# hitbc/panSVR

Hardware: AMD Instinct MI355X
Metric: signal reads realigned/sec (150 bp PE); bit-exact CIGAR vs CPU ref (higher is better)
Workload: dtype u8/int32 (2-bit k-mers, 8-bit DP deltas, 32-bit scores); 1 GPU; configs[1]: 1000000 synthetic 150 bp PE signal read pairs per GPU vs 10000-anchor SV reference (11.8 Mbp), `panSVR aln` hot path; pairs_per_gpu=1000000, engines_per_gpu=1, in_process_rebases=0, index_hbm_bytes=2713674320, index_distribution=every rank uploads its own copy from host memory

## Files before the change

### pansvr_amd/csrc/dp_plan.h

```cpp
#pragma once
#include <stdint.h>
#include <string.h>
#include <algorithm>
#include <vector>
#include "../../include/psvr_engine.h"

#if defined(__HIPCC__)
#define PSVR_HD __host__ __device__ __forceinline__
#else
#define PSVR_HD inline
#endif

namespace psvr {

#define PSVR_DP_NUM_LDS_CLASSES 13
#define PSVR_DP_MAX_LDS (160 * 1024)
PSVR_HD int dp_lds_class_bytes(int cls)
{
	const int t[PSVR_DP_NUM_LDS_CLASSES] = {2048, 4096, 6144, 8192, 12288, 16384, 24576, 32768, 49152, 65536, 98304, 131072, PSVR_DP_MAX_LDS};
	return t[cls];
}
PSVR_HD int dp_lds_class(long long need)
{
	int cls = 0;
// ... 23 lines not shown
}

#define PSVR_DP_STRIP 16
#define PSVR_DP_TINY_MAX 16
#define PSVR_DP_PG_THRESHOLD 4096
static const int kDpWaves = 4;
static const int kDpLongLen = 8000;
static const int kDpMaxSeqLen = 1 << 28;
static const int kDpTinySmallLds = 4096;
PSVR_HD bool dp_band_never_binds(int qlen, int tlen, int w) { return qlen <= w && tlen <= w + 1; }
PSVR_HD int dp_band_w(int qlen, int tlen, int w) { return w < 0 ? (qlen > tlen ? qlen : tlen) : w; }
PSVR_HD int dp_n_col(int qlen, int tlen, int w_in)
{
	int w = dp_band_w(qlen, tlen, w_in);
	int n_col = qlen < tlen ? qlen : tlen;
	n_col = ((n_col < w + 1 ? n_col : w + 1) + 15) / 16 + 1;
	return n_col;
}
PSVR_HD long long dp_reg_lds_need(int qlen, int tlen, int w_in)
{
	return (long long)((qlen + 16 + 15) & ~15) + (long long)(qlen + tlen - 1) * dp_n_col(qlen, tlen, w_in) * 16 + 16;
}
PSVR_HD long long dp_p_bytes(int qlen, int tlen, int w_in)
{
	return ((long long)(qlen + tlen - 1) * dp_n_col(qlen, tlen, w_in) + 1) * 16;
}
PSVR_HD constexpr int dp_lds_kernel_need(int qlen, int tlen, int variant)
{
	int T = (tlen + 15) / 16 * 16, QL = (qlen + 15) / 16 * 16;
	int narr = variant == 0 ? 7 : 5;
	int img = narr * T + T + QL + 16;
	return ((img + 15) & ~15) + 4 * T;
}
static_assert(dp_lds_kernel_need(kDpLongLen, kDpLongLen, 0) <= PSVR_DP_MAX_LDS, "the general kernel's LDS holds every problem that is not long");
PSVR_HD long long dp_hbm_img_off(int qlen, int tlen, int w_in, bool with_cigar)
{
	return with_cigar ? (dp_p_bytes(qlen, tlen, w_in) + 255) & ~255LL : 0;
}
PSVR_HD long long dp_hbm_img_bytes(int qlen, int tlen, int variant)
{
	const long long T = (tlen + 15LL) / 16 * 16, QL = (qlen + 15LL) / 16 * 16;
	return (((variant == 0 ? 8 : 6) * T + QL + 16 + 15) & ~15LL) + 4 * T;
}

struct DpParams {
	int32_t m;
	int32_t q, e, q2, e2;
	int32_t qe_pre;
	int32_t sc_mch, sc_mis, sc_N, m1;
	int32_t w, zdrop, end_bonus, flag;
	int32_t long_thres, long_diff;
	int32_t skip;
	int32_t nowrap_ok;
	int8_t  mat[25];
};
inline bool make_dp_params(const psvr_ksw_params_t *par, int variant, DpParams *P)
{
	memset(P, 0, sizeof *P);
	int m = par->m, q = par->q, e = par->e, q2 = par->q2, e2 = par->e2;
	if (m > 5 || m < 0) return false;
	P->m = m;
	P->qe_pre = q + e;
	memcpy(P->mat, par->mat, 25);
	P->w = par->w, P->zdrop = par->zdrop, P->end_bonus = par->end_bonus, P->flag = par->flag;
	if (variant == 0) {
		if (m <= 1) { P->skip = 1; return true; }
		if (q2 + e2 < q + e) { int t = q; q = q2, q2 = t, t = e, e = e2, e2 = t; }
	} else {
		if (m <= 0) { P->skip = 1; return true; }
		q2 = q, e2 = e;
	}
	P->q = q, P->e = e, P->q2 = q2, P->e2 = e2;
	P->sc_mch = par->mat[0], P->sc_mis = par->mat[1];
	P->sc_N = par->mat[m * m - 1] == 0 ? (int8_t)(-e2) : par->mat[m * m - 1];
	if (variant == 1) P->sc_N = par->mat[m * m - 1] == 0 ? (int8_t)(-e) : par->mat[m * m - 1];
	P->m1 = m - 1;
	int min_sc = par->mat[1];
	for (int t = 1; t < m * m; ++t) min_sc = std::min<int>(min_sc, par->mat[t]);
	if (-min_sc > 2 * (q + e)) { P->skip = 1; return true; }
	{
		int max_sc = par->mat[0];
		for (int t = 1; t < m * m; ++t) max_sc = std::max<int>(max_sc, par->mat[t]);
		int g = std::max(q + e, q2 + e2);
		const bool boundary_is_the_recurrences = e > e2 || (e == e2 && q == q2);
		P->nowrap_ok = (max_sc + 3 * g + std::max(-min_sc, 0) <= 127) && q >= 0 && e >= 0 && q2 >= 0 && e2 >= 0 && boundary_is_the_recurrences;
	}
	if (variant == 0) {
		int lt = e != e2 ? (q2 - q) / (e - e2) - 1 : 0;
		if (q2 + e2 + lt * e2 > q + e + lt * e) ++lt;
		P->long_thres = lt;
		P->long_diff = lt * (e - e2) - (q2 - q) - e2;
	}
	return true;
}
inline bool dp_zdrop_inert(const DpParams &P)
{
	return P.e2 == 0 && (P.zdrop < 0 || P.zdrop >= 2 * P.q2 + (P.qe_pre - (P.q + P.e))) && !(P.flag & PSVR_EZ_EXTZ_ONLY);
}
PSVR_HD bool dp_fast_ok(int flag, int variant) { return variant == 0 && (flag & ~(PSVR_EZ_EXTZ_ONLY | PSVR_EZ_REV_CIGAR | PSVR_EZ_SCORE_ONLY)) == 0; }
PSVR_HD bool dp_tiny_ok(const DpParams &P, bool fast_ok) { return fast_ok && P.nowrap_ok && !P.skip && (P.w < 0 || P.w >= PSVR_DP_TINY_MAX); }

struct DpRoute {
	int kind, need;
	int64_t slab;
};
PSVR_HD DpRoute dp_route(int qlen, int tlen, int w, bool fast_ok, int variant, bool skip, bool tiny_ok, bool team_ok, bool with_cigar)
{
	const bool is_long = qlen > kDpLongLen || tlen > kDpLongLen;
	DpRoute R{1, 0, 0};
	if (skip || (!is_long && (qlen <= 0 || tlen <= 0))) return R;
	const bool dirs = with_cigar || !is_long;
	const int64_t p_slab = dirs ? (dp_p_bytes(qlen, tlen, w) + 255) & ~(int64_t)255 : 0;
	if (!is_long) {
		if (tiny_ok && qlen <= PSVR_DP_TINY_MAX && tlen <= PSVR_DP_TINY_MAX) { R.kind = PSVR_DP_KIND_TINY, R.need = (qlen + tlen - 1) * 512; return R; }
		if (tiny_ok && team_ok && dp_band_never_binds(qlen, tlen, dp_band_w(qlen, tlen, w)) && tlen <= PSVR_DP_STRIP * PSVR_DP_NUM_LDS_CLASSES) {
			R.kind = PSVR_DP_KIND_STRIP, R.need = dp_lds_class_bytes((tlen + PSVR_DP_STRIP - 1) / PSVR_DP_STRIP - 1);
			return R;
		}
		const int T = (tlen + 15) / 16 * 16;
		if (fast_ok && T <= 320) {
			const long long n = dp_reg_lds_need(qlen, tlen, w);
			if (n <= PSVR_DP_PG_THRESHOLD) { R.kind = (T + 63) / 64, R.need = (int)n; return R; }
			R.kind = 5 + (T + 63) / 64, R.need = ((qlen + 16 + 15) & ~15) + 16, R.slab = p_slab;
			return R;
		}
	}
	if (fast_ok) {
		const int wf = dp_band_w(qlen, tlen, w), sh = qlen < tlen ? qlen : tlen;
		const int span = (wf < sh - 1 ? wf : sh - 1) + 33;
		const long long ring_need = ((qlen + 16 + 15) & ~15LL) + ((tlen + 15) & ~15LL) + 16;
		if (span <= 256 && ring_need <= PSVR_DP_MAX_LDS) {
			const bool four = (long long)dp_lds_class_bytes(dp_lds_class(ring_need)) * kDpWaves <= PSVR_DP_MAX_LDS;
			R.kind = span <= 192 ? (four ? PSVR_DP_KIND_RING3 : PSVR_DP_KIND_RING1_3) : (four ? PSVR_DP_KIND_RING4 : PSVR_DP_KIND_RING1_4);
			R.need = (int)ring_need, R.slab = p_slab;
			return R;
		}
	}
	if (is_long) {
		R.kind = PSVR_DP_KIND_HBM;
		R.slab = dp_hbm_img_off(qlen, tlen, w, with_cigar) + ((dp_hbm_img_bytes(qlen, tlen, variant) + 255) & ~(int64_t)255);
		return R;
	}
	R.kind = 0, R.need = dp_lds_kernel_need(qlen, tlen, variant), R.slab = p_slab;
	return R;
}

static constexpr int kDpTeamLanes = 2, kDpTeamCpl = 8;
PSVR_HD int dp_team_lanes(int n_strips16) { return kDpTeamLanes; }
PSVR_HD unsigned long long dp_team_ws_bytes(int qmax, int n_strips16, int lanes, int cpl = kDpTeamCpl)
{
	const int sw = cpl * lanes, pb = 64 / lanes, n_strips = (n_strips16 * 16 + sw - 1) / sw;
	return (unsigned long long)(64 * cpl) * n_strips * (qmax + sw - 1) + (unsigned long long)pb * 20 * (qmax + sw * n_strips + 1);
}
PSVR_HD unsigned long long dp_team_waves(int cls, unsigned long long count) { return (count * dp_team_lanes(cls + 1) + 63) / 64; }
PSVR_HD unsigned long long dp_team_wave_ws(int cls, int qmax) { return dp_team_ws_bytes(qmax > 0 ? qmax : 1, cls + 1, dp_team_lanes(cls + 1)); }
PSVR_HD unsigned long long dp_team_class_ws(int cls, unsigned long long count, int qmax) { return dp_team_waves(cls, count) * dp_team_wave_ws(cls, qmax); }

PSVR_HD int dp_kind_order(int k)
{
	const int t[PSVR_DP_NUM_HOST_KINDS] = {17, 16, 15, 0, 14, 13, 10, 9, 8, 7, 6, 5, 4, 3, 2, 1, PSVR_DP_KIND_TINY, PSVR_DP_KIND_STRIP};
	return t[k];
}
static const int kDpPlanClasses = PSVR_DP_NUM_LDS_CLASSES, kDpPlanKinds = PSVR_DP_NUM_KINDS, kDpPlanTeamKind = PSVR_DP_KIND_STRIP, kDpPlanQBins = 200;
static const int kDpPlanTeam0 = 256;
static const int kDpPlanBuckets = kDpPlanTeam0 + kDpPlanClasses * kDpPlanQBins;
static const int kDpPlanOtherSlots = (kDpPlanKinds - 1) * kDpPlanClasses;
static const int kDpPlanSlots = kDpPlanOtherSlots + kDpPlanClasses * kDpPlanQBins;
static_assert(PSVR_DP_NUM_HOST_KINDS * PSVR_DP_NUM_LDS_CLASSES <= kDpPlanTeam0, "a count per (kind, class) below the team buckets");
PSVR_HD int dp_plan_bucket(int kind, int cls, int qlen)
{
	if (kind == kDpPlanTeamKind) return kDpPlanTeam0 + cls * kDpPlanQBins + (qlen < 1 ? 0 : qlen > kDpPlanQBins ? kDpPlanQBins - 1 : qlen - 1);
	return kind * kDpPlanClasses + cls;
}
PSVR_HD int dp_plan_slot_bucket(int k)
{
	if (k < kDpPlanOtherSlots) return dp_kind_order(PSVR_DP_NUM_HOST_KINDS - PSVR_DP_NUM_KINDS + k / kDpPlanClasses) * kDpPlanClasses + (kDpPlanClasses - 1 - k % kDpPlanClasses);
	k -= kDpPlanOtherSlots;
	return kDpPlanTeam0 + (kDpPlanClasses - 1 - k / kDpPlanQBins) * kDpPlanQBins + (kDpPlanQBins - 1 - k % kDpPlanQBins);
}
inline long long dp_plan_starts(const unsigned int *hist, long long *start)
{
	long long acc = 0;
	for (int b = 0; b < kDpPlanBuckets; ++b) start[b] = 0;
	for (int k = 0; k < kDpPlanSlots; ++k) { const int b = dp_plan_slot_bucket(k); start[b] = acc, acc += hist[b]; }
	return acc;
}

struct DpLaunch {
	int kind, cls;
	long long first, count;
	int qmax;
};
inline std::vector<DpLaunch> dp_launch_list(const unsigned long long *cnt, const unsigned long long *team_cnt, const unsigned long long *team_qmax, bool merge_tiny)
{
	std::vector<DpLaunch> ls;
	long long acc = 0;
	for (int ko = 0; ko < PSVR_DP_NUM_HOST_KINDS; ++ko)
		for (int cls = PSVR_DP_NUM_LDS_CLASSES - 1; cls >= 0; --cls) {
			const int kind = dp_kind_order(ko);
			const bool team = kind == PSVR_DP_KIND_STRIP;
			const long long n = (long long)(team ? team_cnt[cls] : cnt[kind * PSVR_DP_NUM_LDS_CLASSES + cls]);
			if (!n) continue;
			const bool joins = merge_tiny && kind == PSVR_DP_KIND_TINY && !ls.empty() && ls.back().kind == kind &&
			                   (dp_lds_class_bytes(ls.back().cls) > kDpTinySmallLds) == (dp_lds_class_bytes(cls) > kDpTinySmallLds);
			if (joins) ls.back().count += n;
			else ls.push_back(DpLaunch{kind, cls, acc, n, team ? (int)team_qmax[cls] : 0});
			acc += n;
		}
	return ls;
}

struct DpHostPlan {
	std::vector<int32_t> idx;
	std::vector<int64_t> poff;
	std::vector<DpLaunch> launches;
	int64_t slab_bytes = 0, ws_bytes = 0;
};
inline DpHostPlan dp_plan_host(int64_t n, const int32_t *qlen, const int32_t *tlen, const DpParams &P, int variant)
{
	DpHostPlan out;
	const bool fast_ok = dp_fast_ok(P.flag, variant), tiny_ok = dp_tiny_ok(P, fast_ok), with_cigar = !(P.flag & PSVR_EZ_SCORE_ONLY);
	unsigned long long cnt[PSVR_DP_NUM_HOST_KINDS * PSVR_DP_NUM_LDS_CLASSES] = {}, qmax[PSVR_DP_NUM_LDS_CLASSES] = {};
	std::vector<int> slot(n);
	out.poff.assign(n, 0);
	for (int64_t i = 0; i < n; ++i) {
		const DpRoute R = dp_route(qlen[i], tlen[i], P.w, fast_ok, variant, P.skip != 0, tiny_ok, true, with_cigar);
		if (R.slab) out.poff[i] = out.slab_bytes, out.slab_bytes += R.slab;
		const int cls = dp_lds_class(R.need);
		++cnt[slot[i] = R.kind * PSVR_DP_NUM_LDS_CLASSES + cls];
		if (R.kind == PSVR_DP_KIND_STRIP) qmax[cls] = std::max<unsigned long long>(qmax[cls], qlen[i]);
	}
	out.launches = dp_launch_list(cnt, cnt + PSVR_DP_KIND_STRIP * PSVR_DP_NUM_LDS_CLASSES, qmax, false);
	long long at[PSVR_DP_NUM_HOST_KINDS * PSVR_DP_NUM_LDS_CLASSES] = {};
	for (const DpLaunch &L : out.launches) at[L.kind * PSVR_DP_NUM_LDS_CLASSES + L.cls] = L.first;
	out.idx.resize(n);
	for (int64_t i = 0; i < n; ++i) out.idx[at[slot[i]]++] = (int32_t)i;
	for (const DpLaunch &L : out.launches) {
		if (L.kind != PSVR_DP_KIND_STRIP) continue;
		std::stable_sort(out.idx.begin() + L.first, out.idx.begin() + L.first + L.count, [&](int32_t x, int32_t y) { return qlen[x] > qlen[y]; });
		out.ws_bytes += (int64_t)dp_team_class_ws(L.cls, (unsigned long long)L.count, L.qmax);
	}
	return out;
}

}
```

### pansvr_amd/csrc/ksw_kernels.hip

```cpp
#include <hip/hip_runtime.h>
#include <stdint.h>
#include "ksw_device.h"

namespace psvr {

__device__ __forceinline__ void write_ez(psvr_extz_t *o, const EzAcc &a, int n_cigar)
{
	o->max = a.max, o->zdropped = a.zdropped;
	o->max_q = a.max_q, o->max_t = a.max_t;
	o->mqe = a.mqe, o->mqe_t = a.mqe_t;
	o->mte = a.mte, o->mte_q = a.mte_q;
	o->score = a.score, o->n_cigar = n_cigar, o->reach_end = a.reach_end, o->reserved = 0;
}

__device__ __forceinline__ void wave_slot_take(int t, int tlen, const uint8_t *target, int neg_qe, int neg_qe2,
                                               int &u, int &v, int &x, int &y, int &x2, int &y2, int &s, int &H, int &tb)
{
	u = v = x = y = neg_qe, x2 = y2 = neg_qe2, s = 0, H = PSVR_KSW_NEG_INF;
	tb = t < tlen ? target[t] : 0;
}
template <int K, bool RING>
__device__ __forceinline__ void dp_wave_loop(const DpParams &P, const uint8_t *target, int lane, int qlen, int tlen, int w, int rowb, int n_rows,
                                             const uint8_t *QR, uint8_t *Pm, EzAcc &ez)
{
// ... 254 lines not shown
	const int w = dp_band_w(qlen, tlen, P.w);
	const int rowb = uni(dp_n_col(qlen, tlen, P.w) * 16);
	const int n_rows = qlen + tlen - 1;
	const int qimg = (qlen + 16 + 15) & ~15;
	uint8_t *QR = lds;
	uint8_t *Pm = PG ? B.pslab + (uni64(B.p_off[pid]) << B.p_unit_shift) : lds + qimg;
	const int p_end = n_rows * rowb + 16;
	for (int i = lane; i < qimg; i += 64) QR[i] = i < qlen ? query[qlen - 1 - i] : 0;
	if (RING) {
		uint8_t *TG = lds + qimg;
		for (int i = lane; i < tlen; i += 64) TG[i] = target[i];
		dp_wave_loop<K, true>(P, TG, lane, qlen, tlen, w, rowb, n_rows, QR, Pm, ez);
	}
	else if (P.nowrap_ok && dp_band_never_binds(qlen, tlen, w)) dp_lean_loop<K>(P, target, lane, qlen, tlen, rowb, n_rows, QR, Pm, ez);
	else dp_wave_loop<K, false>(P, target, lane, qlen, tlen, w, rowb, n_rows, QR, Pm, ez);
	const int with_cigar = !(P.flag & PSVR_EZ_SCORE_ONLY);
	int n_cigar = 0;
	if (with_cigar) {
		if (PG) __threadfence_block();
		__builtin_amdgcn_wave_barrier();
		int i0, j0;
		if (trace_start(ez, P, qlen, tlen, i0, j0)) {
			uint32_t *stage_end = (uint32_t*)(Pm + p_end);
			n_cigar = traceback(i0, j0, qlen, tlen, w,
				[&](int r, int k) { return PG ? (int)__builtin_nontemporal_load(Pm + (size_t)r * rowb + k) : (int)Pm[r * rowb + k]; },
				[&](int k, uint32_t word) { if (lane == 0) stage_end[-1 - k] = word; });
			if (PG) __threadfence_block();
			__builtin_amdgcn_wave_barrier();
			uint32_t *dst = B.cigar + uni64(out->cigar_off);
			const bool rev = (P.flag & PSVR_EZ_REV_CIGAR) != 0;
			for (int m = lane; m < n_cigar; m += 64) {
				const uint32_t *src = rev ? stage_end - 1 - m : stage_end - n_cigar + m;
				dst[m] = PG ? __builtin_nontemporal_load(src) : *src;
			}
		}
	}
	if (lane == 0) write_ez(out, ez, n_cigar);
}
template <int K, bool PG>
__global__ __launch_bounds__(64 * kDpWaves) void extd2_reg_kernel(DpBatch B, DpParams P) { extd2_wave_body<K, PG, false>(B, P); }
template <int K>
__global__ __launch_bounds__(64 * kDpWaves) void extd2_ring_kernel(DpBatch B, DpParams P) { extd2_wave_body<K, true, true>(B, P); }
template __global__ void extd2_ring_kernel<3>(DpBatch, DpParams);
template __global__ void extd2_ring_kernel<4>(DpBatch, DpParams);
template <int K>
__global__ __launch_bounds__(64) void extd2_ring1_kernel(DpBatch B, DpParams P) { extd2_wave_body<K, true, true, 1>(B, P); }
template __global__ void extd2_ring1_kernel<3>(DpBatch, DpParams);
template __global__ void extd2_ring1_kernel<4>(DpBatch, DpParams);

template __global__ void extd2_reg_kernel<1, false>(DpBatch, DpParams);
template __global__ void extd2_reg_kernel<2, false>(DpBatch, DpParams);
template __global__ void extd2_reg_kernel<1, true>(DpBatch, DpParams);
template __global__ void extd2_reg_kernel<2, true>(DpBatch, DpParams);
template __global__ void extd2_reg_kernel<3, true>(DpBatch, DpParams);
template __global__ void extd2_reg_kernel<4, true>(DpBatch, DpParams);
template __global__ void extd2_reg_kernel<5, true>(DpBatch, DpParams);


__global__ __launch_bounds__(64) void extd2_tiny_kernel(DpBatch B, DpParams P, int max_rows)
{
	extern __shared__ __align__(16) uint32_t tiny_lds[];
	const int lane = threadIdx.x;
	const long long slot = (long long)blockIdx.x * 64 + lane;
	if (slot >= B.n) return;
	uint32_t *W0 = tiny_lds + lane, *W1 = tiny_lds + 16 * 64 + lane;
	uint8_t *PD = (uint8_t *)(tiny_lds + 2 * 16 * 64) + lane;
	const int pid = B.idx[slot];
	const int qlen = B.qlen[pid], tlen = B.tlen[pid];
	psvr_extz_t *out = B.ez + pid;
	EzAcc ez;
	ez.reset();
	if (P.skip || qlen <= 0 || tlen <= 0 || qlen > PSVR_DP_TINY_MAX || tlen > PSVR_DP_TINY_MAX || qlen + tlen - 1 > max_rows) { write_ez(out, ez, 0); return; }
	const uint8_t *query = B.qseq + B.q_off[pid], *target = B.tseq + B.t_off[pid];
	unsigned long long qp = 0, tp = 0;
	for (int i = 0; i < qlen; ++i) qp |= (unsigned long long)(query[i] & 15) << (4 * i);
	for (int i = 0; i < tlen; ++i) tp |= (unsigned long long)(target[i] & 15) << (4 * i);
	const int neg_qe = s8(-P.q - P.e), neg_qe2 = s8(-P.q2 - P.e2);
	const int qe8 = s8(P.q + P.e), qe28 = s8(P.q2 + P.e2);
	const int with_cigar = !(P.flag & PSVR_EZ_SCORE_ONLY);
	auto pack0 = [](int u, int v, int x, int y) { return (uint32_t)(u & 0xff) | (uint32_t)(v & 0xff) << 8 | (uint32_t)(x & 0xff) << 16 | (uint32_t)(y & 0xff) << 24; };
	auto pack1 = [](int x2, int y2, int h) { return (uint32_t)(x2 & 0xff) | (uint32_t)(y2 & 0xff) << 8 | (uint32_t)(h & 0xffff) << 16; };
	for (int t = 0; t < tlen; ++t) {
		W0[t * 64] = pack0(dp_edge_gap(P, t), neg_qe, neg_qe, neg_qe);
		W1[t * 64] = pack1(neg_qe2, neg_qe2, -P.qe_pre);
	}
	const int n_rows = qlen + tlen - 1;
	for (int r = 0; r < n_rows; ++r) {
		const int st0 = max(0, r - qlen + 1), en0 = min(tlen - 1, r);
		const int en1 = dp_diag_en1(st0, en0);
		int x1 = neg_qe, v1 = dp_edge_gap(P, r), x21 = neg_qe2, h1 = 0;
		if (st0 > 0) {
			const uint32_t a = W0[(st0 - 1) * 64], b = W1[(st0 - 1) * 64];
			v1 = s8(a >> 8), x1 = s8(a >> 16), x21 = s8(b), h1 = (int)(int16_t)(b >> 16);
		}
		int bh = (int)0x80000000, H_en0 = 0, H_st0 = 0;
		unsigned bk = 0xffffffffu;
		for (int t = st0; t <= en0; ++t) {
			const uint32_t a = W0[t * 64], b = W1[t * 64];
			const int ut = s8(a), vo = s8(a >> 8), xo = s8(a >> 16), yo = s8(a >> 24), x2o = s8(b), y2o = s8(b >> 8), ho = (int)(int16_t)(b >> 16);
			const int xt1 = x1, vt1 = v1, x2t1 = x21, hl = h1;
			x1 = xo, v1 = vo, x21 = x2o, h1 = ho;
			const int tc = (int)(tp >> (4 * t)) & 15, qc = (int)(qp >> (4 * (r - t))) & 15;
			int sc = tc == qc ? P.sc_mch : P.sc_mis;
			sc = (tc == P.m1 || qc == P.m1) ? P.sc_N : sc;
			int za = xt1 + vt1, zb = yo + ut, za2 = x2t1 + vt1, zb2 = y2o + ut;
			int z = max(max(sc, za), zb);
			z = max(max(z, za2), zb2);
			int d = 4;
			d = za2 == z ? 3 : d;
			d = zb == z ? 2 : d;
			d = za == z ? 1 : d;
			d = sc == z ? 0 : d;
			z = min(z, P.sc_mch);
			const int un = z - vt1, vn = z - ut;
			const int zq = z - P.q, zq2 = z - P.q2;
			za -= zq, zb -= zq, za2 -= zq2, zb2 -= zq2;
			d |= (za > 0 ? 0x08 : 0) | (zb > 0 ? 0x10 : 0) | (za2 > 0 ? 0x20 : 0) | (zb2 > 0 ? 0x40 : 0);
			const int hn = (t == en0 && en0 > 0) ? hl + un : ho + vn;
			W0[t * 64] = pack0(un, vn, max(za, 0) - qe8, max(zb, 0) - qe8);
			W1[t * 64] = pack1(max(za2, 0) - qe28, max(zb2, 0) - qe28, hn);
			if (with_cigar) PD[(r * 16 + t) * 64] = (uint8_t)d;
			if (t == en0) H_en0 = hn;
			if (t == st0) H_st0 = hn;
			const unsigned rank = dp_diag_rank<12>(t, st0, en0, en1);
			if (hn > bh || (hn == bh && rank < bk)) bh = hn, bk = rank;
		}
		const int max_t = dp_rank_col<12>(bk, st0, en0);
		if (ez.end_diagonal(r, qlen, tlen, st0, en0, H_st0, H_en0, bh, max_t, P.zdrop, P.e2)) break;
	}
	int n_cigar = 0;
	if (with_cigar) {
		int i0, j0;
		if (trace_start(ez, P, qlen, tlen, i0, j0)) {
			const int w = dp_band_w(qlen, tlen, P.w);
			n_cigar = traceback(i0, j0, qlen, tlen, w,
				[&](int r, int k) { return (int)PD[(r * 16 + k) * 64]; },
				[&](int k, uint32_t word) { (k < 16 ? W0[k * 64] : W1[(k - 16) * 64]) = word; });
			uint32_t *dst = B.cigar + out->cigar_off;
			const bool rev = (P.flag & PSVR_EZ_REV_CIGAR) != 0;
			for (int m = 0; m < n_cigar; ++m) {
				const int k = rev ? m : n_cigar - 1 - m;
				dst[m] = k < 16 ? W0[k * 64] : W1[(k - 16) * 64];
			}
		}
	}
	write_ez(out, ez, n_cigar);
}

static constexpr int kTeamWaves = 3;
template <int LANES, int CPL, int LEAN>
__global__ __launch_bounds__(64) __attribute__((amdgpu_waves_per_eu(kTeamWaves, 8))) void extd2_team_kernel(DpBatch B, DpParams P, TeamPlan T)
{
	static_assert(CPL == 4 || CPL == 8 || CPL == 16, "columns per lane: direction bytes go out as dwords");
	constexpr int SW = CPL * LANES, PB = 64 / LANES;
	constexpr int kNone = (int)0x80000000;
	const int lane = threadIdx.x, team = lane / LANES, ql = lane % LANES;
	__shared__ int sc_lut[64];
	{
		const int tcode = lane >> 3, qcode = lane & 7;
		sc_lut[lane] = 8 * ((tcode == P.m1 || qcode == P.m1) ? P.sc_N : (tcode == qcode ? P.sc_mch : P.sc_mis)) + 4;
	}
	__builtin_amdgcn_wave_barrier();
	int cls = 0;
	while (cls + 1 < T.n_classes && (int)blockIdx.x >= T.first_block[cls + 1]) ++cls;
	const int n_strips16 = T.n_strips16[cls];
	const long long slot = (long long)((int)blockIdx.x - T.first_block[cls]) * PB + team;
	const bool live = slot < T.count[cls];
	int pid = 0, qlen = 0, tlen = 0;
	if (live) pid = B.idx[T.first_slot[cls] + slot], qlen = B.qlen[pid], tlen = B.tlen[pid];
	const int n_strips = (n_strips16 * 16 + SW - 1) / SW;
	const int qmax = wave_max_i32(qlen > 0 ? qlen : 0);
	const int ksteps = uni(qmax + LANES - 1);
	const int k_last = uni(-wave_max_i32(live && qlen > 0 ? -qlen : (int)0x80000000)) - 1;
	const int R = ksteps, NR = qmax + SW * n_strips + 1;
	const unsigned long long need = dp_team_ws_bytes(qmax, n_strips16, LANES, CPL);
	const unsigned long long base = T.ws_base[cls] + (unsigned long long)((int)blockIdx.x - T.first_block[cls]) * T.ws_need[cls];
	const bool bad_shape = qlen <= 0 || tlen <= 0 || (tlen + SW - 1) / SW > n_strips;
	if (!live) return;
	if (base + need > B.ws_cap && B.err) *B.err = 20;
	if (P.skip || bad_shape || base + need > B.ws_cap) return;
	uint8_t *w0 = B.ws + base;
	const size_t offE = (size_t)(64 * CPL) * n_strips * R;
	uint8_t *const uE0 = w0 + offE, *const uE1 = w0 + offE + (size_t)4 * PB * NR;
	uint8_t *const uD = w0 + offE + (size_t)8 * PB * NR, *const uD23 = uD + (size_t)4 * PB * NR;
	const unsigned lc = (unsigned)CPL * (unsigned)lane, t4 = 4u * (unsigned)team;
	auto at4 = [=](uint8_t *ub, int r) -> int & { return *(int *)(ub + (size_t)r * (4 * PB) + t4); };
	auto atD2 = [=](int r) -> short & { return *(short *)(uD23 + (size_t)r * (4 * PB) + t4); };
	auto atD3 = [=](int r) -> short & { return *(short *)(uD23 + (size_t)r * (4 * PB) + t4 + 2); };
	const uint8_t *query = B.qseq + B.q_off[pid], *target = B.tseq + B.t_off[pid];
	const int with_cigar = !(P.flag & PSVR_EZ_SCORE_ONLY);
	const int neg_qe = s8(-P.q - P.e), neg_qe2 = s8(-P.q2 - P.e2);
	const int x_init = 8 * neg_qe + 3, y_init = 8 * neg_qe + 2, x2_init = 8 * neg_qe2 + 1, y2_init = 8 * neg_qe2;
	const int z_cap = 8 * P.sc_mch + 7;
	const int q_m8 = 8 * P.q - 8, q2_m8 = 8 * P.q2 - 8;
	const int cx = 8 - 8 * s8(P.q + P.e), cx2 = 8 - 8 * s8(P.q2 + P.e2);
	const int long_thres = P.long_thres, ur_short = s8(-P.e), ur_at = s8(P.long_diff), ur_long = s8(-P.e2);
	auto ur_of = [=](int r) { return r == 0 ? neg_qe : r < long_thres ? ur_short : r == long_thres ? ur_at : ur_long; };
	auto h_above = [&](int t) {
		int h = -P.qe_pre;
		const int lt = P.long_thres;
		if (t >= 1) {
			if (lt >= 1) h += t < lt ? t * s8(-P.e) : (lt - 1) * s8(-P.e) + s8(P.long_diff) + (t - lt) * s8(-P.e2);
			else h += t * s8(-P.e2);
		}
		return h;
	};
	auto frank = [](int p) { return (((p << 12) + p) & 0x3fff) ^ 0x3fff; };
	const int ns = (tlen + SW - 1) / SW;
	for (int sv = 0; sv < ns; ++sv) {
		const int s = uni(sv);
		const int c0 = SW * s;
		const int ncols = tlen - c0 < SW ? tlen - c0 : SW;
		const int jb = CPL * ql, cb = c0 + jb;
		const int jx = tlen - 1 - cb;
		const bool own = (unsigned)jx < (unsigned)CPL;
		int U[CPL], V[CPL], X[CPL], Y[CPL], X2[CPL], Y2[CPL], H[CPL], TC[CPL];
		int M[CPL], K[CPL], G[CPL];
		bool inr[CPL];
#pragma unroll
		for (int jj = 0; jj < CPL; ++jj) {
			U[jj] = 8 * ur_of(cb + jj);
			V[jj] = 8 * neg_qe, X[jj] = x_init, Y[jj] = y_init, X2[jj] = x2_init, Y2[jj] = y2_init;
			H[jj] = 8 * h_above(cb + jj);
			inr[jj] = jb + jj < ncols;
			TC[jj] = inr[jj] ? (target[cb + jj] & 7) * 32 : 0;
			M[jj] = kNone, G[jj] = frank(cb + jj);
			const int d = cb + jj - ql;
			const int st = max(0, d - qlen + 1), en = min(tlen - 1, d);
			K[jj] = st + ((en - st) & ~3) - cb;
		}
		(void)M, (void)K, (void)G;
		uint8_t *const Ein = (s & 1) ? uE0 : uE1, *const Eout = (s & 1) ? uE1 : uE0;
		unsigned e_prev = 0;
		unsigned dirw[CPL / 4];
		int d_cur = kNone, out_prev = kNone;
		if (s > 0) {
			e_prev = (unsigned)at4(Ein, 0);
			if (!LEAN && 0 <= ksteps - LANES) d_cur = at4(uD, c0);
		}
		unsigned q_cur = ql == 0 ? query[0] : 0u;
		for (int kv = 0; kv < LANES - 1; ++kv) {
			const int k = uni(kv);
#define TEAM_MASKED 1
#define TEAM_TOPROW 1
#include "ksw_row_step.inc"
#undef TEAM_MASKED
#undef TEAM_TOPROW
		}
		{
			const int k = LANES - 1;
#define TEAM_MASKED 0
#define TEAM_TOPROW 1
#include "ksw_row_step.inc"
#undef TEAM_MASKED
#undef TEAM_TOPROW
		}
		for (int kv = LANES; kv < ksteps; ++kv) {
			const int k = uni(kv);
#define TEAM_MASKED 0
#define TEAM_TOPROW 0
#include "ksw_row_step.inc"
#undef TEAM_MASKED
#undef TEAM_TOPROW
		}
		if (with_cigar) {
			uint32_t *const dst = (uint32_t *)(w0 + (size_t)(s * R + ksteps - 1) * (64 * CPL) + lc);
#pragma unroll
			for (int g = 0; g < CPL / 4; ++g) dst[g] = dirw[g];
		}
		if (LEAN) { __threadfence_block(); continue; }
		if (LANES > 1) {
			const int inc = __builtin_amdgcn_update_dpp(kNone, out_prev, 0x101, 0xf, 0xf, false);
			const int m0 = __builtin_amdgcn_update_dpp(kNone, M[0], 0x101, 0xf, 0xf, false);
			M[CPL - 2] = max(M[CPL - 2], ql == LANES - 1 ? kNone : inc);
			M[CPL - 1] = max(M[CPL - 1], ql == LANES - 1 ? kNone : m0);
		}
#pragma unroll
		for (int jj = 0; jj < CPL; ++jj)
			if (jj > 0 || ql == 0) at4(uD, ksteps - ql + cb + jj) = M[jj];
		__threadfence_block();
	}
}

static constexpr int kFinishWaves = 8;
template <int LANES, int CPL, int LEAN>
__global__ __launch_bounds__(64) __attribute__((amdgpu_waves_per_eu(1, kFinishWaves))) void extd2_team_finish_kernel(DpBatch B, DpParams P, TeamPlan T)
{
	constexpr int SW = CPL * LANES, PB = 64 / LANES, kWinRows = 8;
	__shared__ uint32_t win[kWinRows * (CPL / 4) * 64];
	const int lane = threadIdx.x, team = lane % PB;
	const int tb = (int)((blockIdx.x * 64u + (unsigned)lane) / (unsigned)PB);
	const bool in_grid = tb < T.first_block[T.n_classes];
	int cls = 0;
	while (cls + 1 < T.n_classes && tb >= T.first_block[cls + 1]) ++cls;
	const int n_strips16 = T.n_strips16[cls];
	const long long slot = (long long)(tb - T.first_block[cls]) * PB + team;
	const bool live = in_grid && slot < T.count[cls];
	int pid = 0, qlen = 0, tlen = 0;
	if (live) pid = B.idx[T.first_slot[cls] + slot], qlen = B.qlen[pid], tlen = B.tlen[pid];
	const int n_strips = (n_strips16 * 16 + SW - 1) / SW;
	int qmax = qlen > 0 ? qlen : 0;
#pragma unroll
	for (int d = 1; d < PB; d <<= 1) qmax = max(qmax, __shfl_xor(qmax, d, 64));
	const int ksteps = qmax + LANES - 1;
	const int R = ksteps, NR = qmax + SW * n_strips + 1;
	const unsigned long long need = dp_team_ws_bytes(qmax, n_strips16, LANES, CPL);
	const unsigned long long base = T.ws_base[cls] + (unsigned long long)(tb - T.first_block[cls]) * T.ws_need[cls];
	if (!live) return;
	psvr_extz_t *out = B.ez + pid;
	EzAcc ez;
	ez.reset();
	const bool bad_shape = qlen <= 0 || tlen <= 0 || (tlen + SW - 1) / SW > n_strips;
	if (P.skip || bad_shape || base + need > B.ws_cap) { write_ez(out, ez, 0); return; }
	uint8_t *w0 = B.ws + base;
	const size_t offE = (size_t)(64 * CPL) * n_strips * R;
	uint8_t *const uD = w0 + offE + (size_t)8 * PB * NR, *const uD23 = uD + (size_t)4 * PB * NR;
	const unsigned t4 = 4u * (unsigned)team;
	auto at4 = [=](uint8_t *ub, int r) -> int & { return *(int *)(ub + (size_t)r * (4 * PB) + t4); };
	const int with_cigar = !(P.flag & PSVR_EZ_SCORE_ONLY);
	const int n_rows = qlen + tlen - 1;
	bool stop = false;
	for (int r0 = 0; r0 < n_rows && !stop; r0 += 8) {
		int kd[8], h2[8], h3[8];
#pragma unroll
		for (int u = 0; u < 8; ++u) {
			const int r = min(r0 + u, n_rows - 1);
			const int w23 = at4(uD23, r);
			kd[u] = LEAN ? 0 : at4(uD, r), h2[u] = (int)(short)(w23 & 0xffff), h3[u] = w23 >> 16;
		}
#pragma unroll
		for (int u = 0; u < 8; ++u) {
			const int r = r0 + u;
			if (r >= n_rows || stop) continue;
			const int st0 = max(0, r - qlen + 1), en0 = min(tlen - 1, r);
			const int key = kd[u];
			const int max_H = key >> 16;
			const int H_en0 = h2[u];
			const int max_t = H_en0 == max_H ? en0 : st0 + ((0x7fff - (key & 0xffff)) & 4095);
			if (en0 == tlen - 1 && H_en0 > ez.mte) ez.mte = H_en0, ez.mte_q = r - (((en0 + 16) & ~15) - 1);
			if (r - st0 == qlen - 1 && h3[u] > ez.mqe) ez.mqe = h3[u], ez.mqe_t = st0;
			if (!LEAN && ez.apply_zdrop(max_H, r, max_t, P.zdrop, P.e2)) stop = true;
			else if (r == n_rows - 1) ez.score = H_en0;
		}
	}
	int n_cigar = 0;
	if (with_cigar) {
		int i0, j0;
		if (trace_start(ez, P, qlen, tlen, i0, j0)) {
			const int w = dp_band_w(qlen, tlen, P.w);
			const uint8_t *pb = w0 + team * SW;
			uint32_t *stage = (uint32_t *)(w0 + offE) + team;
			int win_row = -1, win_grp = -1;
			n_cigar = traceback(i0, j0, qlen, tlen, w,
				[&](int r, int k) {
					const int t = k + (max(0, r - qlen + 1) & ~15), row = r - t, grp = t / CPL;
					if (grp != win_grp || row > win_row || row <= win_row - kWinRows) {
						const int s = grp / LANES, gl = grp % LANES;
						const uint8_t *src = pb + (size_t)(s * R + row + gl) * (64 * CPL) + gl * CPL;
						uint32_t tmp[kWinRows][CPL / 4];
#pragma unroll
						for (int d = 0; d < kWinRows; ++d)
#pragma unroll
							for (int u = 0; u < CPL / 4; ++u) tmp[d][u] = d <= row ? ((const uint32_t *)(src - (size_t)d * (64 * CPL)))[u] : 0u;
#pragma unroll
						for (int d = 0; d < kWinRows; ++d)
#pragma unroll
							for (int u = 0; u < CPL / 4; ++u) win[(d * (CPL / 4) + u) * 64 + lane] = tmp[d][u];
						win_row = row, win_grp = grp;
					}
					const int x = t % CPL;
					const unsigned b = (win[((win_row - row) * (CPL / 4) + (x >> 2)) * 64 + lane] >> (8 * (x & 3))) & 0xffu, n = ~b;
					return (int)((4u - ((b >> 4) & 7u)) | ((n >> 3) & 1u) << 3 | ((n >> 2) & 1u) << 4 | ((n >> 1) & 1u) << 5 | (n & 1u) << 6);
				},
				[&](int k, uint32_t word) { stage[(size_t)k * PB] = word; });
			uint32_t *dst = B.cigar + out->cigar_off;
			const bool rev = (P.flag & PSVR_EZ_REV_CIGAR) != 0;
			for (int m = 0; m < n_cigar; ++m) dst[m] = stage[(size_t)(rev ? m : n_cigar - 1 - m) * PB];
		}
	}
	write_ez(out, ez, n_cigar);
}
template __global__ void extd2_team_kernel<kDpTeamLanes, kDpTeamCpl, 0>(DpBatch, DpParams, TeamPlan);
template __global__ void extd2_team_finish_kernel<kDpTeamLanes, kDpTeamCpl, 0>(DpBatch, DpParams, TeamPlan);
template __global__ void extd2_team_kernel<kDpTeamLanes, kDpTeamCpl, 1>(DpBatch, DpParams, TeamPlan);
template __global__ void extd2_team_finish_kernel<kDpTeamLanes, kDpTeamCpl, 1>(DpBatch, DpParams, TeamPlan);

struct GenK {
	int neg_qe, neg_qe2, qe8, qe28;
	int qe;
	uint8_t qe2b, max_scb, qb8;
	int with_cigar, approx_max, right;
};
__device__ __forceinline__ GenK gen_consts(const DpParams &P)
{
	GenK k;
	k.neg_qe = s8(-P.q - P.e), k.neg_qe2 = s8(-P.q2 - P.e2), k.qe8 = s8(P.q + P.e), k.qe28 = s8(P.q2 + P.e2);
	k.qe = P.q + P.e;
	k.qe2b = (uint8_t)((P.q + P.e) * 2), k.max_scb = (uint8_t)(P.mat[0] + (P.q + P.e) * 2), k.qb8 = (uint8_t)P.q;
	k.with_cigar = !(P.flag & PSVR_EZ_SCORE_ONLY), k.approx_max = !!(P.flag & PSVR_EZ_APPROX_MAX);
	k.right = k.with_cigar && (P.flag & PSVR_EZ_RIGHT);
	return k;
}

template <int VAR, class IDX>
struct GenImage {
	static constexpr int NARR = VAR == 0 ? 7 : 5;
	uint8_t *base;
	IDX T, img;
	int8_t *u8, *v8, *x8, *y8, *x28, *y28, *sa;
	uint8_t *sf, *qr;
	int32_t *H;
	__device__ __forceinline__ void place(uint8_t *at, int qlen, int tlen)
	{
		base = at;
		T = ((IDX)tlen + 15) / 16 * 16;
		const IDX QL = ((IDX)qlen + 15) / 16 * 16;
		u8 = (int8_t*)at, v8 = u8 + T, x8 = v8 + T, y8 = x8 + T;
		x28 = VAR == 0 ? y8 + T : nullptr, y28 = VAR == 0 ? x28 + T : nullptr;
		sa = VAR == 0 ? y28 + T : y8 + T;
		sf = (uint8_t*)(sa + T), qr = sf + T;
		img = NARR * T + T + QL + 16;
		H = (int32_t*)(at + ((img + 15) & ~(IDX)15));
	}
// ... 379 lines not shown
```

### pansvr_amd/csrc/ksw_launch.h

```cpp
#pragma once
#include <hip/hip_runtime.h>
#include "ksw_device.h"

namespace psvr {

inline hipError_t dp_launch_kind(int kind, int variant, unsigned count, int lds, hipStream_t stream, const DpBatch &B0, const DpParams &P)
{
	DpBatch B = B0;
	B.n = count, B.lds_per_wave = lds;
	if (kind == PSVR_DP_KIND_TINY) {
		const int max_rows = lds / 512;
		hipLaunchKernelGGL(extd2_tiny_kernel, dim3((count + 63) / 64), dim3(64), (size_t)8192 + (size_t)max_rows * 1024, stream, B, P, max_rows);
		return hipSuccess;
	}
	if (kind == PSVR_DP_KIND_RING1_3 || kind == PSVR_DP_KIND_RING1_4) {
		if (kind == PSVR_DP_KIND_RING1_3) hipLaunchKernelGGL(extd2_ring1_kernel<3>, dim3(count), dim3(64), lds, stream, B, P);
		else hipLaunchKernelGGL(extd2_ring1_kernel<4>, dim3(count), dim3(64), lds, stream, B, P);
		return hipSuccess;
	}
	if (kind == PSVR_DP_KIND_HBM) {
		if (variant == 0) hipLaunchKernelGGL(extd2_hbm_kernel<0>, dim3(count), dim3(64 * kDpHbmWaves), 0, stream, B, P);
		else hipLaunchKernelGGL(extd2_hbm_kernel<1>, dim3(count), dim3(64 * kDpHbmWaves), 0, stream, B, P);
		return hipSuccess;
	}
	const bool reg = kind >= 1;
	dim3 g(reg ? (count + kDpWaves - 1) / kDpWaves : count), b(reg ? 64 * kDpWaves : 64);
	if (reg) lds *= kDpWaves;
	switch (kind) {
	case 1: hipLaunchKernelGGL((extd2_reg_kernel<1, false>), g, b, lds, stream, B, P); break;
	case 2: hipLaunchKernelGGL((extd2_reg_kernel<2, false>), g, b, lds, stream, B, P); break;
	case 3: case 4: case 5: return hipErrorInvalidDeviceFunction;
	case 6: hipLaunchKernelGGL((extd2_reg_kernel<1, true>), g, b, lds, stream, B, P); break;
	case 7: hipLaunchKernelGGL((extd2_reg_kernel<2, true>), g, b, lds, stream, B, P); break;
	case 8: hipLaunchKernelGGL((extd2_reg_kernel<3, true>), g, b, lds, stream, B, P); break;
	case 9: hipLaunchKernelGGL((extd2_reg_kernel<4, true>), g, b, lds, stream, B, P); break;
	case 10: hipLaunchKernelGGL((extd2_reg_kernel<5, true>), g, b, lds, stream, B, P); break;
	case PSVR_DP_KIND_RING3: hipLaunchKernelGGL(extd2_ring_kernel<3>, g, b, lds, stream, B, P); break;
	case PSVR_DP_KIND_RING4: hipLaunchKernelGGL(extd2_ring_kernel<4>, g, b, lds, stream, B, P); break;
	default:
		if (variant == 0) hipLaunchKernelGGL(extd2_lds_kernel<0>, g, b, lds, stream, B, P);
		else hipLaunchKernelGGL(extd2_lds_kernel<1>, g, b, lds, stream, B, P);
	}
	return hipSuccess;
}

struct TeamLaunch {
	TeamPlan T;
	TeamLaunch() { T.n_classes = 0; T.first_block[0] = 0; }
	unsigned long long ws_next = 0;
	void add(int cls, long long first_slot, long long count, int qmax)
	{
		const int c = T.n_classes++;
		T.n_strips16[c] = cls + 1, T.first_slot[c] = first_slot, T.count[c] = count;
		T.first_block[c + 1] = T.first_block[c] + (int)dp_team_waves(cls, (unsigned long long)count);
		T.ws_need[c] = dp_team_wave_ws(cls, qmax);
		T.ws_base[c] = ws_next;
		ws_next += dp_team_class_ws(cls, (unsigned long long)count, qmax);
	}
	void launch_sweep(hipStream_t stream, const DpBatch &B, const DpParams &P, bool lean = false) const
	{
		if (!T.n_classes) return;
		if (lean) hipLaunchKernelGGL((extd2_team_kernel<kDpTeamLanes, kDpTeamCpl, 1>), dim3((unsigned)T.first_block[T.n_classes]), dim3(64), 0, stream, B, P, T);
		else hipLaunchKernelGGL((extd2_team_kernel<kDpTeamLanes, kDpTeamCpl, 0>), dim3((unsigned)T.first_block[T.n_classes]), dim3(64), 0, stream, B, P, T);
	}
	void launch_finish(hipStream_t stream, const DpBatch &B, const DpParams &P, bool lean = false) const
	{
		if (!T.n_classes) return;
		const unsigned blocks = (unsigned)T.first_block[T.n_classes], pb = 64u / kDpTeamLanes;
		if (lean) hipLaunchKernelGGL((extd2_team_finish_kernel<kDpTeamLanes, kDpTeamCpl, 1>), dim3((blocks * pb + 63u) / 64u), dim3(64), 0, stream, B, P, T);
		else hipLaunchKernelGGL((extd2_team_finish_kernel<kDpTeamLanes, kDpTeamCpl, 0>), dim3((blocks * pb + 63u) / 64u), dim3(64), 0, stream, B, P, T);
	}
	void launch(hipStream_t stream, const DpBatch &B, const DpParams &P, bool lean = false) const { launch_sweep(stream, B, P, lean), launch_finish(stream, B, P, lean); }
};
inline hipError_t dp_allow_big_lds()
{
	hipError_t e = hipSuccess;
#define PSVR_ATTR(k) do { hipError_t x = hipFuncSetAttribute((const void *)(k), hipFuncAttributeMaxDynamicSharedMemorySize, PSVR_DP_MAX_LDS); if (x != hipSuccess) e = x; } while (0)
	PSVR_ATTR((extd2_reg_kernel<1, false>)); PSVR_ATTR((extd2_reg_kernel<2, false>));
	PSVR_ATTR(extd2_lds_kernel<0>); PSVR_ATTR(extd2_lds_kernel<1>); PSVR_ATTR(extd2_ring_kernel<3>); PSVR_ATTR(extd2_ring_kernel<4>);
	PSVR_ATTR(extd2_ring1_kernel<3>); PSVR_ATTR(extd2_ring1_kernel<4>);
#undef PSVR_ATTR
	return e;
}

}
```

### pansvr_amd/csrc/ksw_row_step.inc

```
		const int i = k - ql;
		if (with_cigar && k > 0) {
			uint32_t *const dst = (uint32_t *)(w0 + (size_t)(s * R + k - 1) * (64 * CPL) + lc);
#pragma unroll
			for (int g = 0; g < CPL / 4; ++g) dst[g] = dirw[g];
		}
		const bool act = (unsigned)i < (unsigned)qlen;
		const unsigned q_nxt = (unsigned)(i + 1) < (unsigned)qlen ? query[i + 1] : 0u;
		const int qc4 = (int)((q_cur << 2) & 0x1cu);
		int vl = 0, xl = 0, x2l = 0;
		if (LANES > 1) {
			vl = __builtin_amdgcn_update_dpp(0, V[CPL - 1], 0x111, 0xf, 0xf, false), xl = __builtin_amdgcn_update_dpp(0, X[CPL - 1], 0x111, 0xf, 0xf, false);
			x2l = __builtin_amdgcn_update_dpp(0, X2[CPL - 1], 0x111, 0xf, 0xf, false);
			if (!LEAN) {
				const int inc = __builtin_amdgcn_update_dpp(kNone, out_prev, 0x101, 0xf, 0xf, false);
				M[CPL - 2] = max(M[CPL - 2], ql == LANES - 1 ? kNone : inc);
			}
		}
		unsigned e_next = 0;
		int d_nxt = kNone;
		if (s > 0) {
			e_next = (unsigned)at4(Ein, k + 1);
			if (!LEAN && k + 1 <= ksteps - LANES) d_nxt = at4(uD, c0 + k + 1);
		}
		if (ql == 0) {
			if (s > 0) vl = __builtin_amdgcn_sbfe((int)e_prev, 0, 8) << 3, xl = (__builtin_amdgcn_sbfe((int)e_prev, 8, 8) << 3) | 3, x2l = (__builtin_amdgcn_sbfe((int)e_prev, 16, 8) << 3) | 1;
			else vl = 8 * ur_of(i), xl = x_init, x2l = x2_init;
		}
		const int rowc = qlen - 1 - i, rc = rowc - cb, g_row = frank(rowc);
		int acc[CPL];
#pragma unroll
		for (int jj = 0; jj < CPL; ++jj) {
			const int xt1 = jj ? X[jj ? jj - 1 : 0] : xl, vt1 = jj ? V[jj ? jj - 1 : 0] : vl, x2t1 = jj ? X2[jj ? jj - 1 : 0] : x2l;
			const int sc = *(const int *)((const char *)sc_lut + (TC[jj] | qc4));
			const int ut = U[jj];
			int za = xt1 + vt1, zb = Y[jj] + ut, za2 = x2t1 + vt1, zb2 = Y2[jj] + ut;
			int m = max(max(sc, za), zb);
			m = max(max(m, za2), zb2);
			const int z = min(m, z_cap) & ~7;
			const int un = z - vt1, vn = z - ut;
			const int zq = z - q_m8, zq2 = z - q2_m8;
			za -= zq, zb -= zq, za2 -= zq2, zb2 -= zq2;
			int a = m;
			a = (int)__builtin_amdgcn_alignbit((unsigned)a, (unsigned)za, 31);
			a = (int)__builtin_amdgcn_alignbit((unsigned)a, (unsigned)zb, 31);
			a = (int)__builtin_amdgcn_alignbit((unsigned)a, (unsigned)za2, 31);
			a = (int)__builtin_amdgcn_alignbit((unsigned)a, (unsigned)zb2, 31);
			acc[jj] = a;
			const int hn = H[jj] + vn;
			int key = 0;
			if (!LEAN) {
				const int low = ((jj - K[jj]) & 0x4000) | (jj <= rc ? G[jj] : g_row);
				key = (int)((unsigned)hn << 13) | low;
			}
			if (!TEAM_MASKED || act) {
				U[jj] = un, V[jj] = vn;
				X[jj] = max(za, -5) + cx, Y[jj] = max(zb, -6) + cx;
				X2[jj] = max(za2, -7) + cx2, Y2[jj] = max(zb2, -8) + cx2;
				H[jj] = hn;
			}
			if (!LEAN) M[jj] = max(M[jj], (act & inr[jj]) ? key : kNone);
		}
		const int out = LEAN ? 0 : M[0];
		if (!LEAN && ql == 0) at4(uD, c0 + k) = max(out, d_cur);
		if (!LEAN) {
			const int d_in = i + cb + CPL;
			const int st_in = max(0, d_in - qlen + 1), en_in = min(tlen - 1, d_in);
#pragma unroll
			for (int jj = 0; jj + 1 < CPL; ++jj) M[jj] = M[jj + 1], K[jj] = K[jj + 1] + 0;
			M[CPL - 1] = kNone, K[CPL - 1] = st_in + ((en_in - st_in) & ~3) - cb;
		}
#pragma unroll
		for (int g = 0; g < CPL; g += 4) {
			const unsigned lo = __builtin_amdgcn_perm((unsigned)acc[g + 1], (unsigned)acc[g], 0x0c0c0400u);
			const unsigned hi = __builtin_amdgcn_perm((unsigned)acc[g + 3], (unsigned)acc[g + 2], 0x04000c0cu);
			dirw[g >> 2] = lo | hi;
		}
		if (ql == LANES - 1 && s + 1 < ns && act)
			at4(Eout, i) = (int)((((unsigned)V[CPL - 1] >> 3) & 0xffu) | ((((unsigned)X[CPL - 1] >> 3) & 0xffu) << 8) | ((((unsigned)X2[CPL - 1] >> 3) & 0xffu) << 16));
		if (TEAM_TOPROW && i == 0) {
#pragma unroll
			for (int jj = 0; jj < CPL; ++jj) if (inr[jj]) atD2(cb + jj) = (short)(H[jj] >> 3);
		}
		if (own & act) {
			int hx = H[CPL - 1];
#pragma unroll
			for (int u = CPL - 2; u >= 0; --u) hx = jx == u ? H[u] : hx;
			atD2(i + tlen - 1) = (short)(hx >> 3);
		}
		if (k >= k_last && i == qlen - 1) {
#pragma unroll
			for (int jj = 0; jj < CPL; ++jj) if (inr[jj]) atD3(qlen - 1 + cb + jj) = (short)(H[jj] >> 3);
		}
		out_prev = out, e_prev = e_next, d_cur = d_nxt, q_cur = q_nxt;
```

Baseline: 354.2 million reads/s.

## Stage query bases and strip-boundary E records in LDS for the team sweep

The team DP kernel now copies each pair's query bases into dynamic LDS, and when the query fits (at most 78 rows) it also keeps the inter-strip E boundary records in LDS instead of global workspace. Longer queries use a 32-row windowed ring that is refilled from global memory as the sweep advances. The per-row global loads of query[i+1] and E(k+1) in the inner loop become LDS reads, and the in-fits path drops the per-strip block fence. The cost is 12.5 KB of LDS per 64-thread block, which may limit occupancy, plus extra staging loops and the added complexity of the ring indexing.

```diff
diff --git a/pansvr_amd/csrc/dp_plan.h b/pansvr_amd/csrc/dp_plan.h
--- a/pansvr_amd/csrc/dp_plan.h
+++ b/pansvr_amd/csrc/dp_plan.h
@@ -199,6 +199,9 @@
 	const int sw = cpl * lanes, pb = 64 / lanes, n_strips = (n_strips16 * 16 + sw - 1) / sw;
 	return (unsigned long long)(64 * cpl) * n_strips * (qmax + sw - 1) + (unsigned long long)pb * 20 * (qmax + sw * n_strips + 1);
 }
+static constexpr int kDpTeamLdsBytes = 12544, kDpTeamWinRows = 32;
+PSVR_HD constexpr int dp_team_lds_rows(int lanes = kDpTeamLanes) { return (kDpTeamLdsBytes - lanes * (64 / lanes)) / (5 * (64 / lanes)); }
+static_assert(dp_team_lds_rows() == 78 && 2 * kDpTeamWinRows * 5 * (64 / kDpTeamLanes) <= kDpTeamLdsBytes, "the sweep's LDS rows");
 PSVR_HD unsigned long long dp_team_waves(int cls, unsigned long long count) { return (count * dp_team_lanes(cls + 1) + 63) / 64; }
 PSVR_HD unsigned long long dp_team_wave_ws(int cls, int qmax) { return dp_team_ws_bytes(qmax > 0 ? qmax : 1, cls + 1, dp_team_lanes(cls + 1)); }
 PSVR_HD unsigned long long dp_team_class_ws(int cls, unsigned long long count, int qmax) { return dp_team_waves(cls, count) * dp_team_wave_ws(cls, qmax); }
diff --git a/pansvr_amd/csrc/ksw_kernels.hip b/pansvr_amd/csrc/ksw_kernels.hip
--- a/pansvr_amd/csrc/ksw_kernels.hip
+++ b/pansvr_amd/csrc/ksw_kernels.hip
@@ -430,10 +430,12 @@
 __global__ __launch_bounds__(64) __attribute__((amdgpu_waves_per_eu(kTeamWaves, 8))) void extd2_team_kernel(DpBatch B, DpParams P, TeamPlan T)
 {
 	static_assert(CPL == 4 || CPL == 8 || CPL == 16, "columns per lane: direction bytes go out as dwords");
+	static_assert(LANES <= 2 && kDpTeamWinRows % (8 * LANES) == 0, "a lane reads query row i + 1 >= 0 from its LDS slot; a window is whole passes of stage()");
 	constexpr int SW = CPL * LANES, PB = 64 / LANES;
 	constexpr int kNone = (int)0x80000000;
 	const int lane = threadIdx.x, team = lane / LANES, ql = lane % LANES;
 	__shared__ int sc_lut[64];
+	extern __shared__ __align__(16) uint8_t team_lds[];
 	{
 		const int tcode = lane >> 3, qcode = lane & 7;
 		sc_lut[lane] = 8 * ((tcode == P.m1 || qcode == P.m1) ? P.sc_N : (tcode == qcode ? P.sc_mch : P.sc_mis)) + 4;
@@ -466,6 +468,32 @@
 	auto atD2 = [=](int r) -> short & { return *(short *)(uD23 + (size_t)r * (4 * PB) + t4); };
 	auto atD3 = [=](int r) -> short & { return *(short *)(uD23 + (size_t)r * (4 * PB) + t4 + 2); };
 	const uint8_t *query = B.qseq + B.q_off[pid], *target = B.tseq + B.t_off[pid];
+	const int qm = ksteps - (LANES - 1);
+	const bool fits = qm <= dp_team_lds_rows(LANES);
+	const int rmask = fits ? 127 : 2 * kDpTeamWinRows - 1;
+	unsigned *const Es = (unsigned *)team_lds + team;
+	uint8_t *const Qs = team_lds + (size_t)(4 * PB) * (fits ? qm : 2 * kDpTeamWinRows) + team;
+	auto stage = [&](int r0, int n, uint8_t *Ein, bool whole, bool with_e) {
+		asm volatile("" : "+s"(r0));
+		for (int rb = r0; rb < r0 + n; rb += 8 * LANES) {
+			unsigned qv[8], ev[8];
+#pragma unroll
+			for (int u = 0; u < 8; ++u) {
+				const int r = rb + u * LANES + ql;
+				qv[u] = query[min(r, qlen - 1)];
+				ev[u] = with_e ? (unsigned)at4(Ein, min(r, qm - 1)) : 0u;
+			}
+#pragma unroll
+			for (int u = 0; u < 8; ++u) {
+				const int r = rb + u * LANES + ql;
+				if (whole || r < r0 + n) {
+					Qs[(r & rmask) * PB] = (uint8_t)qv[u];
+					if (with_e) Es[(r & rmask) * PB] = ev[u];
+				}
+			}
+		}
+	};
+	if (fits) stage(0, qm + LANES, nullptr, false, false);
 	const int with_cigar = !(P.flag & PSVR_EZ_SCORE_ONLY);
 	const int neg_qe = s8(-P.q - P.e), neg_qe2 = s8(-P.q2 - P.e2);
 	const int x_init = 8 * neg_qe + 3, y_init = 8 * neg_qe + 2, x2_init = 8 * neg_qe2 + 1, y2_init = 8 * neg_qe2;
@@ -496,27 +524,35 @@
 		int M[CPL], K[CPL], G[CPL];
 		bool inr[CPL];
 #pragma unroll
+		for (int jj = 0; jj < CPL; ++jj) TC[jj] = target[min(cb + jj, tlen - 1)];
+#pragma unroll
 		for (int jj = 0; jj < CPL; ++jj) {
 			U[jj] = 8 * ur_of(cb + jj);
 			V[jj] = 8 * neg_qe, X[jj] = x_init, Y[jj] = y_init, X2[jj] = x2_init, Y2[jj] = y2_init;
 			H[jj] = 8 * h_above(cb + jj);
 			inr[jj] = jb + jj < ncols;
-			TC[jj] = inr[jj] ? (target[cb + jj] & 7) * 32 : 0;
 			M[jj] = kNone, G[jj] = frank(cb + jj);
 			const int d = cb + jj - ql;
 			const int st = max(0, d - qlen + 1), en = min(tlen - 1, d);
 			K[jj] = st + ((en - st) & ~3) - cb;
 		}
+#pragma unroll
+		for (int jj = 0; jj < CPL; ++jj) TC[jj] = inr[jj] ? (TC[jj] & 7) * 32 : 0;
 		(void)M, (void)K, (void)G;
 		uint8_t *const Ein = (s & 1) ? uE0 : uE1, *const Eout = (s & 1) ? uE1 : uE0;
+		if (!fits) {
+			if (s > 0) stage(0, kDpTeamWinRows, Ein, true, true);
+			else stage(0, kDpTeamWinRows, nullptr, true, false);
+		}
+		__builtin_amdgcn_fence(__ATOMIC_ACQ_REL, "wavefront");
 		unsigned e_prev = 0;
 		unsigned dirw[CPL / 4];
 		int d_cur = kNone, out_prev = kNone;
 		if (s > 0) {
-			e_prev = (unsigned)at4(Ein, 0);
+			e_prev = Es[0];
 			if (!LEAN && 0 <= ksteps - LANES) d_cur = at4(uD, c0);
 		}
-		unsigned q_cur = ql == 0 ? query[0] : 0u;
+		unsigned q_cur = ql == 0 ? Qs[0] : 0u;
 		for (int kv = 0; kv < LANES - 1; ++kv) {
 			const int k = uni(kv);
 #define TEAM_MASKED 1
@@ -535,6 +571,10 @@
 		}
 		for (int kv = LANES; kv < ksteps; ++kv) {
 			const int k = uni(kv);
+			if (!fits && ((k + 1) & (kDpTeamWinRows - 1)) == 0) {
+				if (s > 0) stage(k + 1, kDpTeamWinRows, Ein, true, true);
+				else stage(k + 1, kDpTeamWinRows, nullptr, true, false);
+			}
 #define TEAM_MASKED 0
 #define TEAM_TOPROW 0
 #include "ksw_row_step.inc"
@@ -546,7 +586,10 @@
 #pragma unroll
 			for (int g = 0; g < CPL / 4; ++g) dst[g] = dirw[g];
 		}
-		if (LEAN) { __threadfence_block(); continue; }
+		if (LEAN) {
+			if (!fits) __threadfence_block();
+			continue;
+		}
 		if (LANES > 1) {
 			const int inc = __builtin_amdgcn_update_dpp(kNone, out_prev, 0x101, 0xf, 0xf, false);
 			const int m0 = __builtin_amdgcn_update_dpp(kNone, M[0], 0x101, 0xf, 0xf, false);
diff --git a/pansvr_amd/csrc/ksw_launch.h b/pansvr_amd/csrc/ksw_launch.h
--- a/pansvr_amd/csrc/ksw_launch.h
+++ b/pansvr_amd/csrc/ksw_launch.h
@@ -60,8 +60,8 @@
 	void launch_sweep(hipStream_t stream, const DpBatch &B, const DpParams &P, bool lean = false) const
 	{
 		if (!T.n_classes) return;
-		if (lean) hipLaunchKernelGGL((extd2_team_kernel<kDpTeamLanes, kDpTeamCpl, 1>), dim3((unsigned)T.first_block[T.n_classes]), dim3(64), 0, stream, B, P, T);
-		else hipLaunchKernelGGL((extd2_team_kernel<kDpTeamLanes, kDpTeamCpl, 0>), dim3((unsigned)T.first_block[T.n_classes]), dim3(64), 0, stream, B, P, T);
+		if (lean) hipLaunchKernelGGL((extd2_team_kernel<kDpTeamLanes, kDpTeamCpl, 1>), dim3((unsigned)T.first_block[T.n_classes]), dim3(64), kDpTeamLdsBytes, stream, B, P, T);
+		else hipLaunchKernelGGL((extd2_team_kernel<kDpTeamLanes, kDpTeamCpl, 0>), dim3((unsigned)T.first_block[T.n_classes]), dim3(64), kDpTeamLdsBytes, stream, B, P, T);
 	}
 	void launch_finish(hipStream_t stream, const DpBatch &B, const DpParams &P, bool lean = false) const
 	{
diff --git a/pansvr_amd/csrc/ksw_row_step.inc b/pansvr_amd/csrc/ksw_row_step.inc
--- a/pansvr_amd/csrc/ksw_row_step.inc
+++ b/pansvr_amd/csrc/ksw_row_step.inc
@@ -5,7 +5,9 @@
 			for (int g = 0; g < CPL / 4; ++g) dst[g] = dirw[g];
 		}
 		const bool act = (unsigned)i < (unsigned)qlen;
-		const unsigned q_nxt = (unsigned)(i + 1) < (unsigned)qlen ? query[i + 1] : 0u;
+		int k1 = k + 1;
+		asm volatile("" : "+s"(k1));
+		const unsigned q_nxt = Qs[((k1 - ql) & rmask) * PB];
 		const int qc4 = (int)((q_cur << 2) & 0x1cu);
 		int vl = 0, xl = 0, x2l = 0;
 		if (LANES > 1) {
@@ -19,7 +21,7 @@
 		unsigned e_next = 0;
 		int d_nxt = kNone;
 		if (s > 0) {
-			e_next = (unsigned)at4(Ein, k + 1);
+			e_next = Es[(min(k1, qm - 1) & rmask) * PB];
 			if (!LEAN && k + 1 <= ksteps - LANES) d_nxt = at4(uD, c0 + k + 1);
 		}
 		if (ql == 0) {
@@ -75,8 +77,11 @@
 			const unsigned hi = __builtin_amdgcn_perm((unsigned)acc[g + 3], (unsigned)acc[g + 2], 0x04000c0cu);
 			dirw[g >> 2] = lo | hi;
 		}
-		if (ql == LANES - 1 && s + 1 < ns && act)
-			at4(Eout, i) = (int)((((unsigned)V[CPL - 1] >> 3) & 0xffu) | ((((unsigned)X[CPL - 1] >> 3) & 0xffu) << 8) | ((((unsigned)X2[CPL - 1] >> 3) & 0xffu) << 16));
+		if (ql == LANES - 1 && s + 1 < ns && act) {
+			const unsigned rec = (((unsigned)V[CPL - 1] >> 3) & 0xffu) | ((((unsigned)X[CPL - 1] >> 3) & 0xffu) << 8) | ((((unsigned)X2[CPL - 1] >> 3) & 0xffu) << 16);
+			if (fits) Es[i * PB] = rec;
+			else at4(Eout, i) = (int)rec;
+		}
 		if (TEAM_TOPROW && i == 0) {
 #pragma unroll
 			for (int jj = 0; jj < CPL; ++jj) if (inr[jj]) atD2(cb + jj) = (short)(H[jj] >> 3);
```

Result: faster. 359.6 million reads/s (median of 6 runs) (+1.5%).
